# adri-romsor/iterative_inference_segm

Measured on AMD Instinct MI355X. Metric: refined images/s (FCN-8 + standard DAE, 10-step iterative inference, 224x224, 11 classes), higher is better.
Workload: dtype f32; 1 GPU; BASELINE configs[1]: FCN-8 + standard DAE (f64c1p2, pool4, trackind, skip), 224x224x3, batch 64/GPU, 10 steps, step 0.1, early stop off; per batch: pred_fcn_fn, val_fn, pred_dae_fn+val_fn, refine, val_fn; global_batch=64, parallelism=dp1

## Files before the change

include/iiseg.h:

```cpp
#ifndef IISEG_H
#define IISEG_H

#include <stdint.h>

#ifdef __cplusplus
extern "C" {
#endif

typedef enum iiseg_status {
    IISEG_OK = 0,
    IISEG_ERR_NULL = -1,
    IISEG_ERR_SHAPE = -2,
    IISEG_ERR_ALIGN = -3,
    IISEG_ERR_LAUNCH = -4,
    IISEG_ERR_UNSUPPORTED = -5
} iiseg_status;

const char* iiseg_strerror(int status);
const char* iiseg_last_hip_error(void);
int iiseg_abi_version(void);
const char* iiseg_target_arch(void);

int iiseg_profile_begin(int capacity);
int iiseg_profile_count(void);
// ... 34 lines not shown
                        const float* pre, const float* pooled, const float* wp, const int32_t* ktab,
                        const float* bias, const float* add, float* out, float* pool_out);

int iiseg_conv_mask_supported(const iiseg_conv_desc* d);
int iiseg_conv_mask_f32(void* stream, const iiseg_conv_desc* d, const float* x1, const float* x2,
                        const float* pre, const float* pooled, const uint8_t* mask_in,
                        const float* wp, const int32_t* ktab, const float* bias, const float* add,
                        float* out, float* pool_out, uint8_t* mask_out);

int iiseg_conv_halo_seam(int on);
int64_t iiseg_conv_halo_seam_launches(void);

int iiseg_conv_bnrelu_supported(const iiseg_conv_desc* d);
int iiseg_conv_bnrelu_f32(void* stream, const iiseg_conv_desc* d, const float* x, int64_t x_bstride,
                          const float* beta, const float* gamma, const float* mean,
                          const float* inv_std, const float* wp, const int32_t* ktab,
                          const float* bias, float* out);

#define IISEG_WINO_INPUT 1u
#define IISEG_WINO_GEMM 2u
#define IISEG_WINO_OUTPUT 4u
#define IISEG_WINO_ALL 7u
#define IISEG_WINO_FUSED 8u
int iiseg_conv_wino_supported(const iiseg_conv_desc* d);
int64_t iiseg_conv_wino_weight_elems(const iiseg_conv_desc* d);
int64_t iiseg_conv_wino_workspace_elems(const iiseg_conv_desc* d);
int iiseg_conv_wino_pack_f32(void* stream, const iiseg_conv_desc* d, const float* w,
                             int64_t stride_o, int64_t stride_c, float* U);
int iiseg_conv_wino_f32(void* stream, const iiseg_conv_desc* d, const float* x1, const float* x2,
                        const float* pre, const float* pooled, const float* U, const float* bias,
                        const float* add, float* workspace, float* out, uint32_t stages);
int iiseg_conv_wino_input_wide(int on);
int iiseg_conv_wino_input_path(const iiseg_conv_desc* d, int mask_bytes);
int iiseg_conv_wino_pool_supported(const iiseg_conv_desc* d);
int iiseg_conv_wino_mask_f32(void* stream, const iiseg_conv_desc* d, const float* x1, const float* x2,
                             const float* pre, const float* pooled, const uint8_t* mask_in,
                             const float* U, const float* bias, const float* add, float* workspace,
                             float* out, float* pool_out, uint8_t* mask_out, uint32_t stages);

int iiseg_conv_wino_bf16_supported(const iiseg_conv_desc* d);
int64_t iiseg_conv_wino_bf16_weight_bytes(const iiseg_conv_desc* d);
int64_t iiseg_conv_wino_bf16_workspace_bytes(const iiseg_conv_desc* d);
int iiseg_conv_wino_bf16_pack(void* stream, const iiseg_conv_desc* d, const float* w,
                              int64_t stride_o, int64_t stride_c, void* U16);
int iiseg_conv_wino_bf16(void* stream, const iiseg_conv_desc* d, const float* x1, const float* x2,
                         const float* pre, const float* pooled, const void* U16, const float* bias,
                         const float* add, void* workspace, float* out, uint32_t stages);

int iiseg_conv_gemm_bf16_supported(const iiseg_conv_desc* d);
int64_t iiseg_conv_gemm_bf16_weight_bytes(const iiseg_conv_desc* d);
int64_t iiseg_conv_gemm_bf16_workspace_bytes(const iiseg_conv_desc* d);
int iiseg_conv_gemm_bf16_pack(void* stream, const iiseg_conv_desc* d, const float* w,
                              int64_t stride_o, int64_t stride_c, void* U16);
int iiseg_conv_gemm_bf16(void* stream, const iiseg_conv_desc* d, const float* x, const void* U16,
                         const float* bias, void* workspace, float* out);

int iiseg_conv_halo_bf16_supported(const iiseg_conv_desc* d);
int64_t iiseg_conv_halo_bf16_weight_bytes(const iiseg_conv_desc* d);
int iiseg_conv_halo_bf16_pack(void* stream, const iiseg_conv_desc* d, const float* w,
                              int64_t stride_o, int64_t stride_c, void* wp16);
int iiseg_conv_halo_bf16(void* stream, const iiseg_conv_desc* d, const float* x1, const float* x2,
                         const float* pre, const float* pooled, const void* wp16, const float* bias,
                         const float* add, float* out, float* pool_out, const uint8_t* mask_in,
                         uint8_t* mask_out);

int iiseg_conv_wino_f64_supported(const iiseg_conv_desc* d);
// ... 335 lines not shown
```

iterative_inference_segm_amd/_lib.py:

```python
import ctypes as C
import os

HERE = os.path.dirname(os.path.abspath(__file__))
LIB_PATH = os.path.join(HERE, 'libiiseg_hip.so')

ABI_VERSION = 34

CONV_RELU = 1
CONV_UNPOOL = 2
CONV_X3 = 8
CONV_TRANSPOSED2 = 4
CONV_ZINS = 16


class ConvDesc(C.Structure):
    _fields_ = [(n, C.c_int32) for n in
                ('B', 'C1', 'C2', 'H', 'W', 'Cout', 'KH', 'KW', 'pad', 'dil',
                 'oy0', 'ox0', 'OH', 'OW', 'AH', 'AW', 'ay0', 'ax0')] + \
               [('flags', C.c_uint32), ('Kpad', C.c_int32), ('Mpad', C.c_int32),
                ('out_ctot', C.c_int32), ('out_c0', C.c_int32),
                ('out_H', C.c_int32), ('out_W', C.c_int32), ('out_y0', C.c_int32),
                ('out_x0', C.c_int32), ('tile_y0', C.c_int32), ('tile_x0', C.c_int32)]


# ... 43 lines not shown


_vp, _i32, _i64, _f32, _f64 = C.c_void_p, C.c_int32, C.c_int64, C.c_float, C.c_double

SIGNATURES = {
    'iiseg_strerror': (C.c_char_p, [C.c_int]),
    'iiseg_last_hip_error': (C.c_char_p, []),
    'iiseg_abi_version': (C.c_int, []),
    'iiseg_profile_begin': (C.c_int, [C.c_int]),
    'iiseg_profile_count': (C.c_int, []),
    'iiseg_profile_end': (C.c_int, [C.POINTER(C.c_float), C.c_int]),
    'iiseg_target_arch': (C.c_char_p, []),
    'iiseg_conv_ktab_entries': (C.c_int, [C.POINTER(ConvDesc)]),
    'iiseg_conv_plan': (C.c_int, [C.POINTER(ConvDesc)]),
    'iiseg_conv_pack_f32': (C.c_int, [_vp, C.POINTER(ConvDesc), _vp, _i64, _i64, _vp, _vp]),
    'iiseg_conv_f32': (C.c_int, [_vp, C.POINTER(ConvDesc)] + [_vp] * 9),
    'iiseg_conv_small_supported': (C.c_int, [C.POINTER(ConvDesc)]),
    'iiseg_conv_pool_supported': (C.c_int, [C.POINTER(ConvDesc)]),
    'iiseg_conv_pool_f32': (C.c_int, [_vp, C.POINTER(ConvDesc)] + [_vp] * 10),
    'iiseg_conv_halo_seam': (C.c_int, [C.c_int]),
    'iiseg_conv_halo_seam_launches': (_i64, []),
    'iiseg_conv_mask_supported': (C.c_int, [C.POINTER(ConvDesc)]),
    'iiseg_conv_mask_f32': (C.c_int, [_vp, C.POINTER(ConvDesc)] + [_vp] * 12),
    'iiseg_conv_bnrelu_supported': (C.c_int, [C.POINTER(ConvDesc)]),
    'iiseg_conv_bnrelu_f32': (C.c_int, [_vp, C.POINTER(ConvDesc), _vp, _i64] + [_vp] * 8),
    'iiseg_conv_wino_supported': (C.c_int, [C.POINTER(ConvDesc)]),
    'iiseg_conv_wino_weight_elems': (_i64, [C.POINTER(ConvDesc)]),
    'iiseg_conv_wino_workspace_elems': (_i64, [C.POINTER(ConvDesc)]),
    'iiseg_conv_wino_pack_f32': (C.c_int, [_vp, C.POINTER(ConvDesc), _vp, _i64, _i64, _vp]),
    'iiseg_conv_wino_f32': (C.c_int, [_vp, C.POINTER(ConvDesc)] + [_vp] * 9 + [C.c_uint32]),
    'iiseg_conv_wino_pool_supported': (C.c_int, [C.POINTER(ConvDesc)]),
    'iiseg_conv_wino_input_wide': (C.c_int, [C.c_int]),
    'iiseg_conv_wino_input_path': (C.c_int, [C.POINTER(ConvDesc), C.c_int]),
    'iiseg_conv_wino_mask_f32': (C.c_int, [_vp, C.POINTER(ConvDesc)] + [_vp] * 12 + [C.c_uint32]),
    'iiseg_conv_wino_bf16_supported': (C.c_int, [C.POINTER(ConvDesc)]),
    'iiseg_conv_wino_bf16_weight_bytes': (_i64, [C.POINTER(ConvDesc)]),
    'iiseg_conv_wino_bf16_workspace_bytes': (_i64, [C.POINTER(ConvDesc)]),
    'iiseg_conv_wino_bf16_pack': (C.c_int, [_vp, C.POINTER(ConvDesc), _vp, _i64, _i64, _vp]),
    'iiseg_conv_wino_bf16': (C.c_int, [_vp, C.POINTER(ConvDesc)] + [_vp] * 9 + [C.c_uint32]),
    'iiseg_conv_gemm_bf16_supported': (C.c_int, [C.POINTER(ConvDesc)]),
    'iiseg_conv_gemm_bf16_weight_bytes': (_i64, [C.POINTER(ConvDesc)]),
    'iiseg_conv_gemm_bf16_workspace_bytes': (_i64, [C.POINTER(ConvDesc)]),
    'iiseg_conv_gemm_bf16_pack': (C.c_int, [_vp, C.POINTER(ConvDesc), _vp, _i64, _i64, _vp]),
    'iiseg_conv_gemm_bf16': (C.c_int, [_vp, C.POINTER(ConvDesc)] + [_vp] * 5),
    'iiseg_conv_halo_bf16_supported': (C.c_int, [C.POINTER(ConvDesc)]),
    'iiseg_conv_halo_bf16_weight_bytes': (_i64, [C.POINTER(ConvDesc)]),
    'iiseg_conv_halo_bf16_pack': (C.c_int, [_vp, C.POINTER(ConvDesc), _vp, _i64, _i64, _vp]),
    'iiseg_conv_halo_bf16': (C.c_int, [_vp, C.POINTER(ConvDesc)] + [_vp] * 11),
    'iiseg_conv_wino_f64_supported': (C.c_int, [C.POINTER(ConvDesc)]),
    'iiseg_conv_wino_f64_weight_elems': (_i64, [C.POINTER(ConvDesc)]),
    'iiseg_conv_wino_f64_workspace_elems': (_i64, [C.POINTER(ConvDesc)]),
    'iiseg_conv_wino_pack_f64': (C.c_int, [_vp, C.POINTER(ConvDesc), _vp, _i64, _i64, _vp]),
    'iiseg_conv_wino_f64': (C.c_int, [_vp, C.POINTER(ConvDesc)] + [_vp] * 9),
    'iiseg_conv_c8_supported': (C.c_int, [C.POINTER(ConvDesc)]),
    'iiseg_conv_c8_is_flat': (C.c_int, [C.POINTER(ConvDesc)]),
    'iiseg_conv_c8_force_tiling': (C.c_int, [C.c_int, C.c_int, C.c_int]),
    'iiseg_conv_c8_tiling': (C.c_int, [C.POINTER(ConvDesc), C.c_int, C.POINTER(C.c_int32)]),
    'iiseg_conv_c8': (C.c_int, [_vp, C.POINTER(ConvDesc)] + [_vp] * 6 + [_i32, _vp, _i32, _vp, _vp]),
    'iiseg_conv_c8_slice': (C.c_int, [_vp, C.POINTER(ConvDesc), _vp, _i32] + [_vp] * 5 + [_i32, _vp, _i32, _vp, _vp]),
    'iiseg_unpool_c8': (C.c_int, [_vp] * 4 + [C.c_int] * 7),
    'iiseg_conv_c8_m16_supported': (C.c_int, [C.POINTER(ConvDesc)]),
    'iiseg_conv_c8_m16': (C.c_int, [_vp, C.POINTER(ConvDesc), _vp, _i32] + [_vp] * 6 + [_i32]),
    'iiseg_conv_c8_m16_workspace_bytes': (_i64, [C.POINTER(ConvDesc)]),
    'iiseg_conv_c8_m16_ws': (C.c_int, [_vp, C.POINTER(ConvDesc), _vp, _i32] + [_vp] * 6 + [_i32, _vp, _i64, _vp, _vp, _f64] + [_vp] * 4 + [_i32]),
    'iiseg_conv1x1_c8_weight_bytes': (_i64, [C.c_int, C.c_int]),
    'iiseg_conv1x1_c8_pack': (C.c_int, [_vp, _vp, _i64, _i64, C.c_int, C.c_int, C.c_int, _vp]),
# ... 145 lines not shown
```

iterative_inference_segm_amd/csrc/conv_wino.hip:

```cpp
#include <hip/hip_runtime.h>
#include <stdint.h>
#include <stdlib.h>
#include <atomic>
#include <type_traits>
#include "iiseg.h"
#include "common.h"
#include "conv_common.h"

using namespace iiseg;

namespace {

struct WinoParams {
    const float* x1;
    const float* x2;
    const float* pre;
    const float* pooled;
    const uint8_t* mask_in;
    int h2, w2;
    const float* U;
    const float* bias;
    const float* add;
    float* V;
    float* M;
// ... 574 lines not shown
                for (int j = 0; j < TN; ++j)
                    acc[i][j] = __builtin_amdgcn_mfma_f32_32x32x2f32(a[ch & 1][i], b[ch & 1][j],
                                                                     acc[i][j], 0, 0, 0);
            if constexpr (ch == 0) {
                if (more) WINO_STAGE(kt + NBUF - 1, sbuf)
            }
            __builtin_amdgcn_sched_barrier(0);
        });
        if (NBUF == 3 && more) {
            WINO_WAIT_ONE_STAGE_IN_FLIGHT()
        } else {
            asm volatile("s_waitcnt vmcnt(0)" ::: "memory");
        }
        __syncthreads();
        if (++buf == NBUF) buf = 0;
    }
#undef WINO_STAGE
#undef WINO_WAIT_ONE_STAGE_IN_FLIGHT

    float* Mx = p.M + (size_t)xi * p.Mpad * p.Tpad;
#pragma unroll
    for (int j = 0; j < TN; ++j) {
        const int t = t0 + wn * WTN + j * 32 + l31;
#pragma unroll
        for (int i = 0; i < TM; ++i)
#pragma unroll
            for (int r = 0; r < 16; ++r) {
                const int co = m0 + wm * WTM + i * 32 + (r & 3) + 8 * (r >> 2) + 4 * lh;
                Mx[(size_t)co * p.Tpad + t] = acc[i][j][r];
            }
    }
}

template <int BM, int BN, int WM, int WN, int BK, int MINW>
__global__ __launch_bounds__(WM * WN * 64, MINW) void wino_fused_kernel(const WinoParams p) {
    constexpr int NCH = BK / 2;
    constexpr int WTM = BM / WM, WTN = BN / WN;
    constexpr int TM = WTM / 32, TN = WTN / 32;
    constexpr int NT = WM * WN * 64;
    constexpr int AV = BK * BM / 4, BV = BK * BN / 4;
    constexpr int APT = AV / NT, BPT = BV / NT;
    static_assert(AV % NT == 0 && BV % NT == 0, "tile config");

    __shared__ __attribute__((aligned(16))) float As[2][BK][BM];
    __shared__ __attribute__((aligned(16))) float Bs[2][BK][BN];

    int tt, mt;
    tile_of_block(blockIdx.x, gridDim.x, p.n_ttiles, p.n_mtiles, tt, mt);
    const int m0 = mt * BM, t0 = tt * BN;
    const int tid = threadIdx.x, lane = tid & 63, wave = tid >> 6;
    const int wm = wave / WN, wn = wave % WN;
    const int l31 = lane & 31, lh = lane >> 5;
    const int nkt = p.Kc / BK;
    const size_t ustride = (size_t)p.Kc * p.Mpad, vstride = (size_t)p.Kc * p.Tpad;
    const int ubytes = p.Kc * p.Mpad * 4, vbytes = p.Kc * p.Tpad * 4;

#define WINO_STAGE(XI, KT, BUF)                                                                    \
    {                                                                                              \
        const __amdgpu_buffer_rsrc_t ar = mk_rsrc(p.U + (size_t)(XI) * ustride, ubytes);           \
        const __amdgpu_buffer_rsrc_t br = mk_rsrc(p.V + (size_t)(XI) * vstride, vbytes);           \
        static_for<0, APT>([&](auto J) __attribute__((always_inline)) {                            \
            constexpr int j = decltype(J)::value;                                                  \
            const int f = j * NT + tid;                                                            \
            const int row = f / (BM / 4), c4 = f % (BM / 4);                                       \
            __builtin_amdgcn_raw_ptr_buffer_load_lds(                                              \
                ar, (__attribute__((address_space(3))) void*)(&As[BUF][0][0] + (j * NT + wave * 64) * 4), \
                16, (int)(4u * (unsigned)(((KT) * BK + row) * p.Mpad + m0 + c4 * 4)), 0, 0, 0);    \
        });                                                                                        \
        static_for<0, BPT>([&](auto J) __attribute__((always_inline)) {                            \
            constexpr int j = decltype(J)::value;                                                  \
            const int f = j * NT + tid;                                                            \
            const int row = f / (BN / 4), c4 = f % (BN / 4);                                       \
            __builtin_amdgcn_raw_ptr_buffer_load_lds(                                              \
                br, (__attribute__((address_space(3))) void*)(&Bs[BUF][0][0] + (j * NT + wave * 64) * 4), \
                16, (int)(4u * (unsigned)(((KT) * BK + row) * p.Tpad + t0 + c4 * 4)), 0, 0, 0);    \
        });                                                                                        \
    }

    f32x16 acc[TM][TN], Y[4][TM][TN];
#pragma unroll
    for (int i = 0; i < TM; ++i)
#pragma unroll
        for (int j = 0; j < TN; ++j)
#pragma unroll
            for (int r = 0; r < 16; ++r) {
                acc[i][j][r] = 0.f;
                Y[0][i][j][r] = Y[1][i][j][r] = Y[2][i][j][r] = Y[3][i][j][r] = 0.f;
            }

    WINO_STAGE(0, 0, 0)
    asm volatile("s_waitcnt vmcnt(0)" ::: "memory");
    __syncthreads();

    int xi = 0, kt = 0;
    const int total = 16 * nkt;
    for (int s = 0; s < total; ++s) {
        const int buf = s & 1;
        int nxi = xi, nkt1 = kt + 1;
        if (nkt1 == nkt) { nkt1 = 0; ++nxi; }
        const bool more = s + 1 < total;
        float a[2][TM], b[2][TN];
#pragma unroll
        for (int i = 0; i < TM; ++i) a[0][i] = As[buf][lh][wm * WTM + i * 32 + l31];
#pragma unroll
        for (int j = 0; j < TN; ++j) b[0][j] = Bs[buf][lh][wn * WTN + j * 32 + l31];
        static_for<0, NCH>([&](auto CH) __attribute__((always_inline)) {
            constexpr int ch = decltype(CH)::value;
            if constexpr (ch + 1 < NCH) {
                const int kk = (ch + 1) * 2 + lh;
#pragma unroll
                for (int i = 0; i < TM; ++i) a[(ch + 1) & 1][i] = As[buf][kk][wm * WTM + i * 32 + l31];
#pragma unroll
                for (int j = 0; j < TN; ++j) b[(ch + 1) & 1][j] = Bs[buf][kk][wn * WTN + j * 32 + l31];
            }
#pragma unroll
            for (int i = 0; i < TM; ++i)
#pragma unroll
                for (int j = 0; j < TN; ++j)
                    acc[i][j] = __builtin_amdgcn_mfma_f32_32x32x2f32(a[ch & 1][i], b[ch & 1][j],
                                                                     acc[i][j], 0, 0, 0);
            if constexpr (ch == 0) {
                if (more) WINO_STAGE(nxi, nkt1, buf ^ 1)
            }
            __builtin_amdgcn_sched_barrier(0);
        });
        if (nkt1 == 0) {
            const int wi = xi >> 2, wj = xi & 3;
            const float r0 = wi < 3 ? 1.f : 0.f, r1 = wi == 0 ? 0.f : (wi == 1 ? 1.f : -1.f);
            const float c0 = wj < 3 ? 1.f : 0.f, c1 = wj == 0 ? 0.f : (wj == 1 ? 1.f : -1.f);
            const float k00 = r0 * c0, k01 = r0 * c1, k10 = r1 * c0, k11 = r1 * c1;
#define WINO_FOLD(Q, KQ)                                                                            \
            if ((KQ) != 0.f) {                                                                      \
                _Pragma("unroll") for (int i = 0; i < TM; ++i)                                      \
                _Pragma("unroll") for (int j = 0; j < TN; ++j)                                      \
                _Pragma("unroll") for (int r = 0; r < 16; ++r)                                      \
                    Y[Q][i][j][r] = fmaf((KQ), acc[i][j][r], Y[Q][i][j][r]);                        \
            }
            WINO_FOLD(0, k00)
            WINO_FOLD(1, k01)
            WINO_FOLD(2, k10)
            WINO_FOLD(3, k11)
#undef WINO_FOLD
#pragma unroll
            for (int i = 0; i < TM; ++i)
#pragma unroll
                for (int j = 0; j < TN; ++j)
#pragma unroll
                    for (int r = 0; r < 16; ++r) acc[i][j][r] = 0.f;
        }
        xi = nxi;
        kt = nkt1;
        asm volatile("s_waitcnt vmcnt(0)" ::: "memory");
        __syncthreads();
    }
#undef WINO_STAGE

    typedef float f32x2u __attribute__((ext_vector_type(2), aligned(4)));
    const int ntt = p.nty * p.ntx;
    const size_t OPL = (size_t)p.out_H * p.out_W, APL = (size_t)p.AH * p.AW;
    float* Lbias = &As[0][0][0];
    for (int f = tid; f < BM; f += NT) Lbias[f] = (p.bias && m0 + f < p.Cout) ? p.bias[m0 + f] : 0.f;
    __syncthreads();
    float bias_r[TM][16];
#pragma unroll
    for (int i = 0; i < TM; ++i)
#pragma unroll
        for (int r = 0; r < 16; ++r) bias_r[i][r] = Lbias[wm * WTM + i * 32 + (r & 3) + 8 * (r >> 2) + 4 * lh];
#pragma unroll
    for (int j = 0; j < TN; ++j) {
        const int t = t0 + wn * WTN + j * 32 + l31;
        if (t >= p.T) continue;
        const int b = t / ntt;
        const int rr = t - b * ntt;
        const int tyl = rr / p.ntx, txl = rr - tyl * p.ntx;
        const int wy = p.ty0 + 2 * tyl - p.oy0, wx = p.tx0 + 2 * txl - p.ox0;
        const bool rok[2] = {(unsigned)wy < (unsigned)p.OH, (unsigned)(wy + 1) < (unsigned)p.OH};
        const bool cok[2] = {(unsigned)wx < (unsigned)p.OW, (unsigned)(wx + 1) < (unsigned)p.OW};
        const bool pair = cok[0] && cok[1];
        const bool whole = p.pool && rok[1] && cok[1];
        float* ob = p.out ? p.out + ((size_t)b * p.out_ctot + p.out_c0) * OPL +
                                (ptrdiff_t)(p.out_y0 + wy) * p.out_W + p.out_x0 + wx
                          : nullptr;
        const float* ab = p.add ? p.add + (size_t)b * p.Cout * APL +
                                      (ptrdiff_t)(p.ay0 + wy) * p.AW + p.ax0 + wx
                                : nullptr;
#pragma unroll
        for (int i = 0; i < TM; ++i)
// ... 139 lines not shown
        d->pad < 0 || d->OH <= 0 || d->OW <= 0 || d->oy0 < 0 || d->ox0 < 0)
        return IISEG_ERR_SHAPE;
    const int fullH = d->H + 2 * d->pad - 2, fullW = d->W + 2 * d->pad - 2;
    if (d->oy0 + d->OH > fullH || d->ox0 + d->OW > fullW) return IISEG_ERR_SHAPE;
    if ((d->C1 + d->C2) % 16) return IISEG_ERR_UNSUPPORTED;
    g.Kc = d->C1 + d->C2;
    g.bm = d->Cout > 128 ? 256 : (d->Cout > 64 ? 128 : 64);
    g.Mpad = round_up(d->Cout, g.bm);
    if ((d->tile_y0 | d->tile_x0) & ~1) return IISEG_ERR_SHAPE;
    g.ty0 = d->oy0 - ((d->oy0 - d->tile_y0) & 1);
    g.tx0 = d->ox0 - ((d->ox0 - d->tile_x0) & 1);
    g.nty = (d->oy0 + d->OH - g.ty0 + 1) >> 1;
    g.ntx = (d->ox0 + d->OW - g.tx0 + 1) >> 1;
    const int64_t T = (int64_t)d->B * g.nty * g.ntx;
    const int64_t Tpad = (T + 127) / 128 * 128;
    if (Tpad * g.Kc * 4 >= (int64_t)1 << 31 || (int64_t)g.Kc * g.Mpad * 4 >= (int64_t)1 << 31)
        return IISEG_ERR_UNSUPPORTED;
    g.T = (int)T;
    g.Tpad = (int)Tpad;
    return IISEG_OK;
}

std::atomic<int> g_input_wide{-1};

int input_wide_setting() {
    int v = g_input_wide.load();
    if (v < 0) {
        v = getenv("IISEG_WINO_INPUT_WIDE") ? (atoi(getenv("IISEG_WINO_INPUT_WIDE")) != 0) : 1;
        g_input_wide.store(v);
    }
    return v;
}

bool iw_fits(const WinoParams& p, int nt) {
    const int NC = 2 * p.ntx + 2;
    for (int t0 = 0; t0 < p.T; t0 += 4 * nt) {
        const int t1 = t0 + 4 * nt < p.T ? t0 + 4 * nt : p.T;
        if ((int64_t)iw_chunk(t0, t1, p.ntx, p.nty).NR * NC > (int64_t)IW_E * nt) return false;
    }
    return true;
}

int ilds_nt(const WinoParams& p);
constexpr int IW_NT = 256;

int iw_shape(const WinoParams& p, bool unpool, bool mb) {
    const int setting = input_wide_setting();
    if (!setting || (unpool && !mb)) return 0;
    if (setting != 2) {
        if (p.T < 4096) return 0;
        const int lnt = mb ? 0 : ilds_nt(p);
        if (lnt && (p.nty * p.ntx) % lnt == 0) return 0;
    }
    const int64_t HW = (int64_t)p.H * p.W, cmax = p.C1 > p.C2 ? p.C1 : p.C2;
    if (HW > (1 << IW_PBITS) || (int64_t)p.B * cmax * HW >= (int64_t)1 << 30) return 0;
    const int64_t waves1 = ((int64_t)p.T + 255) / 256 * p.Kc;
    int ch = 8;
    if (p.Kc % 32 == 0 && waves1 / 32 >= 2048) ch = 32;
    else if (waves1 / 16 >= 2048) ch = 16;
    return iw_fits(p, IW_NT) ? ch : 0;
}

int ilds_nt(const WinoParams& p) {
    static const int lds = getenv("IISEG_WINO_INPUT_LDS") ? atoi(getenv("IISEG_WINO_INPUT_LDS")) : 1;
    const int ntt = p.nty * p.ntx;
    int nt = 0;
// ... 18 lines not shown
    }
    const int nt = ilds_nt(p);
    const int ntt = p.nty * p.ntx;
    if (nt) {
        const int chunks = (ntt + nt - 1) / nt;
        const dim3 g2(p.B * chunks, p.Kc / ILDS_CH);
#define WINO_ILDS(U, N, ...) IISEG_LAUNCH((wino_input_lds_kernel<U, N, ##__VA_ARGS__>), g2, dim3(N), 0, s, p, chunks)
        if (mb) { if (nt == 256) WINO_ILDS(true, 256, true); else if (nt == 128) WINO_ILDS(true, 128, true); else WINO_ILDS(true, 64, true); }
        else if (unpool) { if (nt == 256) WINO_ILDS(true, 256); else if (nt == 128) WINO_ILDS(true, 128); else WINO_ILDS(true, 64); }
        else { if (nt == 256) WINO_ILDS(false, 256); else if (nt == 128) WINO_ILDS(false, 128); else WINO_ILDS(false, 64); }
#undef WINO_ILDS
        return;
    }
    const int nc = unpool ? ICH / 2 : ICH;
    const dim3 grid((p.T + 255) / 256, (p.Kc + nc - 1) / nc), block(256);
    if (!unpool) {
        IISEG_LAUNCH((wino_input_kernel<false, 0, 0>), grid, block, 0, s, p);
        return;
    }
    const int py = (p.ty0 - p.pad) & 1, px = (p.tx0 - p.pad) & 1;
    if (mb) {
        if (py && px) IISEG_LAUNCH((wino_input_kernel<true, 1, 1, true>), grid, block, 0, s, p);
        else if (py) IISEG_LAUNCH((wino_input_kernel<true, 1, 0, true>), grid, block, 0, s, p);
        else if (px) IISEG_LAUNCH((wino_input_kernel<true, 0, 1, true>), grid, block, 0, s, p);
        else IISEG_LAUNCH((wino_input_kernel<true, 0, 0, true>), grid, block, 0, s, p);
        return;
    }
    if (py && px) IISEG_LAUNCH((wino_input_kernel<true, 1, 1>), grid, block, 0, s, p);
    else if (py) IISEG_LAUNCH((wino_input_kernel<true, 1, 0>), grid, block, 0, s, p);
    else if (px) IISEG_LAUNCH((wino_input_kernel<true, 0, 1>), grid, block, 0, s, p);
    else IISEG_LAUNCH((wino_input_kernel<true, 0, 0>), grid, block, 0, s, p);
}

}

int iiseg_wino_output_launch(hipStream_t s, const iiseg_conv_desc* d, const float* M, int Mpad,
                             int Tpad, const float* bias, const float* add, float* out) {
    WinoParams p = {};
    p.M = const_cast<float*>(M);
    p.bias = bias; p.add = add; p.out = out;
    p.B = d->B; p.Cout = d->Cout; p.pad = d->pad;
    p.oy0 = d->oy0; p.ox0 = d->ox0; p.OH = d->OH; p.OW = d->OW;
    p.ty0 = d->oy0 - ((d->oy0 - d->tile_y0) & 1);
    p.tx0 = d->ox0 - ((d->ox0 - d->tile_x0) & 1);
    p.nty = (d->oy0 + d->OH - p.ty0 + 1) >> 1;
    p.ntx = (d->ox0 + d->OW - p.tx0 + 1) >> 1;
    p.T = d->B * p.nty * p.ntx;
    p.Tpad = Tpad; p.Mpad = Mpad;
    p.AH = d->AH; p.AW = d->AW; p.ay0 = d->ay0; p.ax0 = d->ax0;
    p.relu = (d->flags & IISEG_CONV_RELU) ? 1 : 0;
    p.out_ctot = d->out_ctot > 0 ? d->out_ctot : d->Cout;
    p.out_c0 = d->out_ctot > 0 ? d->out_c0 : 0;
    p.out_H = d->out_H > 0 ? d->out_H : d->OH;
    p.out_W = d->out_H > 0 ? d->out_W : d->OW;
    p.out_y0 = d->out_H > 0 ? d->out_y0 : 0;
    p.out_x0 = d->out_H > 0 ? d->out_x0 : 0;
    IISEG_LAUNCH(wino_output_kernel, dim3((p.T + 255) / 256, (d->Cout + OCH - 1) / OCH),
                       dim3(256), 0, s, p);
    return iiseg_check_launch();
}

extern "C" int iiseg_conv_wino_supported(const iiseg_conv_desc* d) {
    WinoGeom g;
    return wino_geom(d, g) == IISEG_OK ? 1 : 0;
}

extern "C" int iiseg_conv_wino_input_wide(int on) {
    if (on >= 0) g_input_wide.store(on > 1 ? 2 : on);
    return input_wide_setting();
}

extern "C" int iiseg_conv_wino_input_path(const iiseg_conv_desc* d, int mask_bytes) {
    WinoGeom g;
    const int st = wino_geom(d, g);
    if (st) return st;
    WinoParams p = {};
    const bool unpool = (d->flags & IISEG_CONV_UNPOOL) != 0;
    if (mask_bytes && !unpool) return IISEG_ERR_UNSUPPORTED;
    p.B = d->B; p.C1 = d->C1; p.C2 = d->C2; p.H = d->H; p.W = d->W;
    p.nty = g.nty; p.ntx = g.ntx; p.T = g.T; p.Tpad = g.Tpad; p.Kc = g.Kc;
    if (iw_shape(p, unpool, mask_bytes != 0)) return 2;
    return ilds_nt(p) ? 1 : 0;
}

extern "C" int64_t iiseg_conv_wino_weight_elems(const iiseg_conv_desc* d) {
    WinoGeom g;
    if (wino_geom(d, g) != IISEG_OK) return 0;
    return (int64_t)16 * g.Kc * g.Mpad;
}

extern "C" int64_t iiseg_conv_wino_workspace_elems(const iiseg_conv_desc* d) {
    WinoGeom g;
    if (wino_geom(d, g) != IISEG_OK) return 0;
    return (int64_t)16 * g.Tpad * ((int64_t)g.Kc + g.Mpad);
}

extern "C" int iiseg_conv_wino_pack_f32(void* stream, const iiseg_conv_desc* d, const float* w,
                                        int64_t stride_o, int64_t stride_c, float* U) {
    WinoGeom g;
    const int st = wino_geom(d, g);
    if (st) return st;
    if (!w || !U) return IISEG_ERR_NULL;
    const int64_t n = (int64_t)g.Kc * g.Mpad;
    const int grid = (int)((n + 255) / 256 < 4096 ? (n + 255) / 256 : 4096);
    IISEG_LAUNCH(wino_weight_kernel, dim3(grid), dim3(256), 0, (hipStream_t)stream, w,
                       stride_o, stride_c, U, d->C1 + d->C2, d->Cout, g.Kc, g.Mpad);
    return iiseg_check_launch();
}

static bool wino_pool_ok(const iiseg_conv_desc* d) {
    WinoGeom g;
    if (wino_geom(d, g) != IISEG_OK) return false;
    const int fullH = d->H + 2 * d->pad - 2, fullW = d->W + 2 * d->pad - 2;
    if ((d->tile_y0 | d->tile_x0 | d->oy0 | d->ox0) & 1) return false;
    if ((d->OH & 1) && d->oy0 + d->OH != fullH) return false;
// ... 35 lines not shown
    p.U = U;
    p.bias = bias;
    p.add = add;
    p.V = workspace;
    p.M = workspace + (size_t)16 * g.Kc * g.Tpad;
    p.out = out;
    p.B = d->B; p.C1 = d->C1; p.C2 = d->C2; p.H = d->H; p.W = d->W;
    p.Cout = d->Cout; p.pad = d->pad;
    p.oy0 = d->oy0; p.ox0 = d->ox0; p.OH = d->OH; p.OW = d->OW;
    p.ty0 = g.ty0; p.tx0 = g.tx0; p.nty = g.nty; p.ntx = g.ntx;
    p.T = g.T; p.Tpad = g.Tpad; p.Kc = g.Kc; p.Mpad = g.Mpad;
    p.AH = d->AH; p.AW = d->AW; p.ay0 = d->ay0; p.ax0 = d->ax0;
    if (add && (d->ay0 < 0 || d->ax0 < 0 || d->ay0 + d->OH > d->AH || d->ax0 + d->OW > d->AW))
        return IISEG_ERR_SHAPE;
    p.relu = (d->flags & IISEG_CONV_RELU) ? 1 : 0;
    p.out_ctot = d->out_ctot > 0 ? d->out_ctot : d->Cout;
    p.out_c0 = d->out_ctot > 0 ? d->out_c0 : 0;
    if (p.out_c0 < 0 || p.out_c0 + d->Cout > p.out_ctot) return IISEG_ERR_SHAPE;
    p.out_H = d->out_H > 0 ? d->out_H : d->OH;
    p.out_W = d->out_H > 0 ? d->out_W : d->OW;
    p.out_y0 = d->out_H > 0 ? d->out_y0 : 0;
    p.out_x0 = d->out_H > 0 ? d->out_x0 : 0;
    if (p.out_y0 < 0 || p.out_x0 < 0 || p.out_y0 + d->OH > p.out_H || p.out_x0 + d->OW > p.out_W)
        return IISEG_ERR_SHAPE;
    p.n_ttiles = g.Tpad / 128;
    p.n_mtiles = g.Mpad / g.bm;
    hipStream_t s = (hipStream_t)stream;
    const int tb = (g.T + 255) / 256;
    if (stages & IISEG_WINO_FUSED) {
        if (g.Kc % 32) return IISEG_ERR_UNSUPPORTED;
        if (stages & IISEG_WINO_INPUT)
            launch_wino_input(s, p, unpool);
        if (stages & IISEG_WINO_GEMM) {
            if (g.bm == 64) {
                p.n_mtiles = g.Mpad / 64;
                IISEG_LAUNCH((wino_fused_kernel<64, 128, 1, 4, 32, 2>),
                                   dim3(p.n_ttiles * p.n_mtiles), dim3(256), 0, s, p);
                return iiseg_check_launch();
            }
            p.n_mtiles = g.Mpad / 128;
            const int w0 = p.n_ttiles * p.n_mtiles, w2 = (g.Tpad / 64) * p.n_mtiles;
            const double cost0 = (w0 + 255) / 256, cost2 = 0.5 * 1.03 * ((w2 + 255) / 256);
            static const int bk64 = getenv("IISEG_WINO_FUSED_BK") ? atoi(getenv("IISEG_WINO_FUSED_BK")) == 64 : 0;
            const bool big = bk64 && g.Kc % 64 == 0;
            if (g.Kc <= 128 || cost2 < cost0) {
                p.n_ttiles = g.Tpad / 64;
                if (big)
                    IISEG_LAUNCH((wino_fused_kernel<128, 64, 2, 2, 64, 2>),
                                       dim3(p.n_ttiles * p.n_mtiles), dim3(256), 0, s, p);
                else
                IISEG_LAUNCH((wino_fused_kernel<128, 64, 2, 2, 32, 2>),
                                   dim3(p.n_ttiles * p.n_mtiles), dim3(256), 0, s, p);
            } else if (big)
                IISEG_LAUNCH((wino_fused_kernel<128, 128, 2, 4, 64, 2>),
                                   dim3(p.n_ttiles * p.n_mtiles), dim3(512), 0, s, p);
            else
            IISEG_LAUNCH((wino_fused_kernel<128, 128, 2, 4, 32, 2>),
                               dim3(p.n_ttiles * p.n_mtiles), dim3(512), 0, s, p);
        }
        return iiseg_check_launch();
    }
    if (stages & IISEG_WINO_INPUT)
        launch_wino_input(s, p, unpool);
    const int grid = 16 * p.n_ttiles * p.n_mtiles;
    if (stages & IISEG_WINO_GEMM) {
        static const int nbuf = getenv("IISEG_WINO_NBUF") ? atoi(getenv("IISEG_WINO_NBUF")) : 2;
        int bm = g.bm;
        if (bm == 64) {
            IISEG_LAUNCH((wino_gemm_kernel<64, 128, 1, 4, 2>), dim3(grid), dim3(256), 0, s, p);
            bm = 0;
        }
        if (bm == 256) {
            const int w256 = grid, w128 = 2 * grid;
            if (0.5 * 1.06 * ((w128 + 255) / 256) < (double)((w256 + 255) / 256)) bm = 128;
        }
        const int grid2 = bm ? 16 * p.n_ttiles * (g.Mpad / bm) : 0;
        if (bm) p.n_mtiles = g.Mpad / bm;
        static const int bk32 = getenv("IISEG_WINO_GEMM_BK") ? atoi(getenv("IISEG_WINO_GEMM_BK")) == 32 : 0;
        if (bm && bk32 && g.Kc % 32 == 0 && nbuf != 3) {
            if (bm == 256)
                IISEG_LAUNCH((wino_gemm_kernel<256, 128, 4, 2, 2, 32>), dim3(grid), dim3(512), 0, s, p);
            else
                IISEG_LAUNCH((wino_gemm_kernel<128, 128, 2, 2, 2, 32>), dim3(grid2), dim3(256), 0, s, p);
        } else
        if (bm == 0) {
        } else if (bm == 256 && nbuf == 3)
            IISEG_LAUNCH((wino_gemm_kernel<256, 128, 4, 2, 3>), dim3(grid), dim3(512), 0, s, p);
        else if (bm == 256)
            IISEG_LAUNCH((wino_gemm_kernel<256, 128, 4, 2, 2>), dim3(grid), dim3(512), 0, s, p);
        else if (nbuf == 3)
            IISEG_LAUNCH((wino_gemm_kernel<128, 128, 2, 2, 3>), dim3(grid2), dim3(256), 0, s, p);
// ... 169 lines not shown
```

iterative_inference_segm_amd/ops.py:

```python
import collections
import ctypes as C
import os

import torch

from . import _lib
from ._lib import ConvDesc, DeconvDesc, CONV_RELU, CONV_UNPOOL, CONV_TRANSPOSED2, CONV_X3, CONV_ZINS, check

CONV_PROFILE = None
CONV_PROFILE_INFO = None
KERNEL_BYTES = {}

_SUFFIX = {torch.float32: 'f32', torch.float64: 'f64'}

WINO_MIN_CIN = int(os.environ.get('IISEG_WINO_MIN_CIN', '128'))
WINO_F64 = os.environ.get('IISEG_WINO_F64', '1') != '0'
WINO_F64_MIN_CIN = int(os.environ.get('IISEG_WINO_F64_MIN_CIN', '128'))
WINO_F64_MIN_COUT = int(os.environ.get('IISEG_WINO_F64_MIN_COUT', '128'))
WINO_MIN_COUT = int(os.environ.get('IISEG_WINO_MIN_COUT', '128'))
WINO_FUSED_MAX_CIN = int(os.environ.get('IISEG_WINO_FUSED_MAX_CIN', '256'))
POOL_FUSE = os.environ.get('IISEG_POOL_FUSE', '1') != '0'
WINO_POOL_FUSE = os.environ.get('IISEG_WINO_POOL_FUSE', '1') != '0'
F64_POOL_FUSE = os.environ.get('IISEG_F64_POOL_FUSE', '1') != '0'
F64_MASKS = os.environ.get('IISEG_F64_MASKS', '1') != '0'
# ... 16 lines not shown
        with open(BF16_PICKS_FILE) as f:
            return {k: v for k, v in json.load(f).get('picks', {}).items() if v in ('wino', 'halo')}
    except OSError:
        return {}


BF16_PICKS = _load_bf16_picks()
BF16_TIMES = {}


def _bf16_static_pick(Cin, OW):
    fill = OW / (32.0 * ((OW + 31) // 32))
    return 'wino' if (Cin >= 1024 or fill < 0.7) else 'halo'


C8_M16 = os.environ.get('IISEG_C8_M16', '1') != '0'
BF16_UPCONV1 = os.environ.get('IISEG_BF16_UPCONV1', '0') != '0'
BF16_WINO_MIN_COUT = int(os.environ.get('IISEG_BF16_WINO_MIN_COUT', '256'))
_SCRATCH_KINDS = {'f32': torch.float32, 'f64': torch.float64, 'bn': torch.float64, 'm16': torch.uint8}
_scratch = {}
_ws_tag = [0]


def halo_seam(on=None):
    return bool(_lib.load().iiseg_conv_halo_seam(-1 if on is None else int(bool(on))))


def halo_seam_launches():
    return int(_lib.load().iiseg_conv_halo_seam_launches())


def wino_input_wide(on=None, force=False):
    return bool(_lib.load().iiseg_conv_wino_input_wide(-1 if on is None else (2 if on and force else int(bool(on)))))


class workspace_tag:

    def __init__(self, tag):
        self.tag, self.prev = tag, None

    def __enter__(self):
        self.prev, _ws_tag[0] = _ws_tag[0], self.tag
        return self

    def __exit__(self, *exc):
        _ws_tag[0] = self.prev
        return False


def current_workspace_tag():
    return _ws_tag[0]


def _workspace(kind, n, device):
    key = (kind, device, _ws_tag[0])
    ws = _scratch.get(key)
    if ws is None or ws.numel() < n:
        _scratch[key] = None
        ws = _scratch[key] = torch.empty(int(n), dtype=_SCRATCH_KINDS[kind], device=device)
    return ws


def drop_workspaces(tag):
    for key in [k for k in _scratch if k[2] == tag]:
        _scratch.pop(key, None)

# ... 1672 lines not shown
```

Before: 529.9 images/s.

## Add configurable multi-buffer ring and precomputed DMA offsets to fused Winograd kernel

Measured after the change: 532.6 images/s (median of 6 runs). Within noise of the previous version (+0.5%).

```diff
diff --git a/include/iiseg.h b/include/iiseg.h
--- a/include/iiseg.h
+++ b/include/iiseg.h
@@ -90,6 +90,7 @@
                         const float* add, float* workspace, float* out, uint32_t stages);
 int iiseg_conv_wino_input_wide(int on);
 int iiseg_conv_wino_input_path(const iiseg_conv_desc* d, int mask_bytes);
+int iiseg_conv_wino_fused_ring(int ring);
 int iiseg_conv_wino_pool_supported(const iiseg_conv_desc* d);
 int iiseg_conv_wino_mask_f32(void* stream, const iiseg_conv_desc* d, const float* x1, const float* x2,
                              const float* pre, const float* pooled, const uint8_t* mask_in,
diff --git a/iterative_inference_segm_amd/_lib.py b/iterative_inference_segm_amd/_lib.py
--- a/iterative_inference_segm_amd/_lib.py
+++ b/iterative_inference_segm_amd/_lib.py
@@ -99,6 +99,7 @@
     'iiseg_conv_wino_pool_supported': (C.c_int, [C.POINTER(ConvDesc)]),
     'iiseg_conv_wino_input_wide': (C.c_int, [C.c_int]),
     'iiseg_conv_wino_input_path': (C.c_int, [C.POINTER(ConvDesc), C.c_int]),
+    'iiseg_conv_wino_fused_ring': (C.c_int, [C.c_int]),
     'iiseg_conv_wino_mask_f32': (C.c_int, [_vp, C.POINTER(ConvDesc)] + [_vp] * 12 + [C.c_uint32]),
     'iiseg_conv_wino_bf16_supported': (C.c_int, [C.POINTER(ConvDesc)]),
     'iiseg_conv_wino_bf16_weight_bytes': (_i64, [C.POINTER(ConvDesc)]),
diff --git a/iterative_inference_segm_amd/csrc/conv_wino.hip b/iterative_inference_segm_amd/csrc/conv_wino.hip
--- a/iterative_inference_segm_amd/csrc/conv_wino.hip
+++ b/iterative_inference_segm_amd/csrc/conv_wino.hip
@@ -630,7 +630,7 @@
     }
 }
 
-template <int BM, int BN, int WM, int WN, int BK, int MINW>
+template <int BM, int BN, int WM, int WN, int BK, int MINW, int NBUF = 2>
 __global__ __launch_bounds__(WM * WN * 64, MINW) void wino_fused_kernel(const WinoParams p) {
     constexpr int NCH = BK / 2;
     constexpr int WTM = BM / WM, WTN = BN / WN;
@@ -639,9 +639,11 @@
     constexpr int AV = BK * BM / 4, BV = BK * BN / 4;
     constexpr int APT = AV / NT, BPT = BV / NT;
     static_assert(AV % NT == 0 && BV % NT == 0, "tile config");
-
-    __shared__ __attribute__((aligned(16))) float As[2][BK][BM];
-    __shared__ __attribute__((aligned(16))) float Bs[2][BK][BN];
+    constexpr int OPS = APT + BPT;
+    static_assert(NBUF >= 2 && NBUF - 1 <= 16 && (NBUF - 2) * OPS <= 63, "ring config");
+
+    __shared__ __attribute__((aligned(16))) float As[NBUF][BK][BM];
+    __shared__ __attribute__((aligned(16))) float Bs[NBUF][BK][BN];
 
     int tt, mt;
     tile_of_block(blockIdx.x, gridDim.x, p.n_ttiles, p.n_mtiles, tt, mt);
@@ -653,26 +655,30 @@
     const size_t ustride = (size_t)p.Kc * p.Mpad, vstride = (size_t)p.Kc * p.Tpad;
     const int ubytes = p.Kc * p.Mpad * 4, vbytes = p.Kc * p.Tpad * 4;
 
+    unsigned avo[APT], bvo[BPT];
+#pragma unroll
+    for (int j = 0; j < APT; ++j) {
+        const int f = j * NT + tid;
+        avo[j] = 4u * (unsigned)((f / (BM / 4)) * p.Mpad + m0 + (f % (BM / 4)) * 4);
+    }
+#pragma unroll
+    for (int j = 0; j < BPT; ++j) {
+        const int f = j * NT + tid;
+        bvo[j] = 4u * (unsigned)((f / (BN / 4)) * p.Tpad + t0 + (f % (BN / 4)) * 4);
+    }
+    const unsigned lds_a = __builtin_amdgcn_readfirstlane(lds_addr(&As[0][0][0]) + (unsigned)wave * 1024u);
+    const unsigned lds_b = __builtin_amdgcn_readfirstlane(lds_addr(&Bs[0][0][0]) + (unsigned)wave * 1024u);
 #define WINO_STAGE(XI, KT, BUF)                                                                    \
     {                                                                                              \
-        const __amdgpu_buffer_rsrc_t ar = mk_rsrc(p.U + (size_t)(XI) * ustride, ubytes);           \
-        const __amdgpu_buffer_rsrc_t br = mk_rsrc(p.V + (size_t)(XI) * vstride, vbytes);           \
-        static_for<0, APT>([&](auto J) __attribute__((always_inline)) {                            \
-            constexpr int j = decltype(J)::value;                                                  \
-            const int f = j * NT + tid;                                                            \
-            const int row = f / (BM / 4), c4 = f % (BM / 4);                                       \
-            __builtin_amdgcn_raw_ptr_buffer_load_lds(                                              \
-                ar, (__attribute__((address_space(3))) void*)(&As[BUF][0][0] + (j * NT + wave * 64) * 4), \
-                16, (int)(4u * (unsigned)(((KT) * BK + row) * p.Mpad + m0 + c4 * 4)), 0, 0, 0);    \
-        });                                                                                        \
-        static_for<0, BPT>([&](auto J) __attribute__((always_inline)) {                            \
-            constexpr int j = decltype(J)::value;                                                  \
-            const int f = j * NT + tid;                                                            \
-            const int row = f / (BN / 4), c4 = f % (BN / 4);                                       \
-            __builtin_amdgcn_raw_ptr_buffer_load_lds(                                              \
-                br, (__attribute__((address_space(3))) void*)(&Bs[BUF][0][0] + (j * NT + wave * 64) * 4), \
-                16, (int)(4u * (unsigned)(((KT) * BK + row) * p.Tpad + t0 + c4 * 4)), 0, 0, 0);    \
-        });                                                                                        \
+        const i32x4s ar = mk_srsrc(p.U + (size_t)(XI) * ustride, (unsigned)ubytes);                \
+        const i32x4s br = mk_srsrc(p.V + (size_t)(XI) * vstride, (unsigned)vbytes);                \
+        const unsigned soa = __builtin_amdgcn_readfirstlane(4u * (unsigned)((KT) * BK * p.Mpad));  \
+        const unsigned sob = __builtin_amdgcn_readfirstlane(4u * (unsigned)((KT) * BK * p.Tpad));  \
+        const unsigned la = __builtin_amdgcn_readfirstlane(lds_a + (unsigned)(BUF) * (BK * BM * 4)); \
+        const unsigned lb = __builtin_amdgcn_readfirstlane(lds_b + (unsigned)(BUF) * (BK * BN * 4)); \
+        asm volatile("s_nop 4");      \
+        _Pragma("unroll") for (int j = 0; j < APT; ++j) dma16(ar, la + j * NT * 16, avo[j], soa);  \
+        _Pragma("unroll") for (int j = 0; j < BPT; ++j) dma16(br, lb + j * NT * 16, bvo[j], sob);  \
     }
 
     f32x16 acc[TM][TN], Y[4][TM][TN];
@@ -686,17 +692,25 @@
                 Y[0][i][j][r] = Y[1][i][j][r] = Y[2][i][j][r] = Y[3][i][j][r] = 0.f;
             }
 
-    WINO_STAGE(0, 0, 0)
-    asm volatile("s_waitcnt vmcnt(0)" ::: "memory");
+    int sxi = 0, skt = 0;
+#define WINO_STAGE_NEXT(BUF)                                                                       \
+    {                                                                                              \
+        WINO_STAGE(sxi, skt, BUF)                                                                  \
+        if (++skt == nkt) { skt = 0; ++sxi; }                                                      \
+    }
+    static_for<0, NBUF - 1>([&](auto SLOT) __attribute__((always_inline)) {
+        constexpr int slot = decltype(SLOT)::value;
+        WINO_STAGE_NEXT(slot)
+    });
+    asm volatile("s_waitcnt vmcnt(%0)" ::"n"((NBUF - 2) * OPS) : "memory");
     __syncthreads();
 
-    int xi = 0, kt = 0;
+    int xi = 0, kt = 0, buf = 0;
     const int total = 16 * nkt;
     for (int s = 0; s < total; ++s) {
-        const int buf = s & 1;
-        int nxi = xi, nkt1 = kt + 1;
-        if (nkt1 == nkt) { nkt1 = 0; ++nxi; }
-        const bool more = s + 1 < total;
+        const bool more = s + NBUF - 1 < total;
+        int sbuf = buf + NBUF - 1;
+        if (sbuf >= NBUF) sbuf -= NBUF;
         float a[2][TM], b[2][TN];
 #pragma unroll
         for (int i = 0; i < TM; ++i) a[0][i] = As[buf][lh][wm * WTM + i * 32 + l31];
@@ -718,11 +732,11 @@
                     acc[i][j] = __builtin_amdgcn_mfma_f32_32x32x2f32(a[ch & 1][i], b[ch & 1][j],
                                                                      acc[i][j], 0, 0, 0);
             if constexpr (ch == 0) {
-                if (more) WINO_STAGE(nxi, nkt1, buf ^ 1)
+                if (more) WINO_STAGE_NEXT(sbuf)
             }
             __builtin_amdgcn_sched_barrier(0);
         });
-        if (nkt1 == 0) {
+        if (++kt == nkt) {
             const int wi = xi >> 2, wj = xi & 3;
             const float r0 = wi < 3 ? 1.f : 0.f, r1 = wi == 0 ? 0.f : (wi == 1 ? 1.f : -1.f);
             const float c0 = wj < 3 ? 1.f : 0.f, c1 = wj == 0 ? 0.f : (wj == 1 ? 1.f : -1.f);
@@ -745,12 +759,15 @@
                 for (int j = 0; j < TN; ++j)
 #pragma unroll
                     for (int r = 0; r < 16; ++r) acc[i][j][r] = 0.f;
-        }
-        xi = nxi;
-        kt = nkt1;
-        asm volatile("s_waitcnt vmcnt(0)" ::: "memory");
+            kt = 0;
+            ++xi;
+        }
+        if (NBUF > 2 && more) asm volatile("s_waitcnt vmcnt(%0)" ::"n"((NBUF - 2) * OPS) : "memory");
+        else asm volatile("s_waitcnt vmcnt(0)" ::: "memory");
         __syncthreads();
-    }
+        if (++buf == NBUF) buf = 0;
+    }
+#undef WINO_STAGE_NEXT
 #undef WINO_STAGE
 
     typedef float f32x2u __attribute__((ext_vector_type(2), aligned(4)));
@@ -956,6 +973,20 @@
     return v;
 }
 
+std::atomic<int> g_fused_ring{-1};
+
+int fused_ring_setting() {
+    int v = g_fused_ring.load();
+    if (v < 0) {
+        v = getenv("IISEG_WINO_FUSED_RING") ? atoi(getenv("IISEG_WINO_FUSED_RING")) : 0;
+        if (v < 2 || v > 4) v = 0;
+        g_fused_ring.store(v);
+    }
+    return v;
+}
+
+int fused_ring_form(int setting) { return setting ? setting : 2; }
+
 bool iw_fits(const WinoParams& p, int nt) {
     const int NC = 2 * p.ntx + 2;
     for (int t0 = 0; t0 < p.T; t0 += 4 * nt) {
@@ -1076,6 +1107,11 @@
 extern "C" int iiseg_conv_wino_input_wide(int on) {
     if (on >= 0) g_input_wide.store(on > 1 ? 2 : on);
     return input_wide_setting();
+}
+
+extern "C" int iiseg_conv_wino_fused_ring(int ring) {
+    if (ring >= 0) g_fused_ring.store(ring >= 2 && ring <= 4 ? ring : 0);
+    return fused_ring_setting();
 }
 
 extern "C" int iiseg_conv_wino_input_path(const iiseg_conv_desc* d, int mask_bytes) {
@@ -1190,10 +1226,17 @@
         if (stages & IISEG_WINO_INPUT)
             launch_wino_input(s, p, unpool);
         if (stages & IISEG_WINO_GEMM) {
+#define WINO_FUSED(BM, BN, WM, WN, NTHR)                                                           \
+            {                                                                                      \
+                const int ring = fused_ring_form(fused_ring_setting());                            \
+                const dim3 fg(p.n_ttiles * p.n_mtiles);                                            \
+                if (ring == 3) IISEG_LAUNCH((wino_fused_kernel<BM, BN, WM, WN, 32, 2, 3>), fg, dim3(NTHR), 0, s, p); \
+                else if (ring == 4) IISEG_LAUNCH((wino_fused_kernel<BM, BN, WM, WN, 16, 2, 4>), fg, dim3(NTHR), 0, s, p); \
+                else IISEG_LAUNCH((wino_fused_kernel<BM, BN, WM, WN, 32, 2>), fg, dim3(NTHR), 0, s, p); \
+            }
             if (g.bm == 64) {
                 p.n_mtiles = g.Mpad / 64;
-                IISEG_LAUNCH((wino_fused_kernel<64, 128, 1, 4, 32, 2>),
-                                   dim3(p.n_ttiles * p.n_mtiles), dim3(256), 0, s, p);
+                WINO_FUSED(64, 128, 1, 4, 256)
                 return iiseg_check_launch();
             }
             p.n_mtiles = g.Mpad / 128;
@@ -1207,14 +1250,13 @@
                     IISEG_LAUNCH((wino_fused_kernel<128, 64, 2, 2, 64, 2>),
                                        dim3(p.n_ttiles * p.n_mtiles), dim3(256), 0, s, p);
                 else
-                IISEG_LAUNCH((wino_fused_kernel<128, 64, 2, 2, 32, 2>),
-                                   dim3(p.n_ttiles * p.n_mtiles), dim3(256), 0, s, p);
+                    WINO_FUSED(128, 64, 2, 2, 256)
             } else if (big)
                 IISEG_LAUNCH((wino_fused_kernel<128, 128, 2, 4, 64, 2>),
                                    dim3(p.n_ttiles * p.n_mtiles), dim3(512), 0, s, p);
             else
-            IISEG_LAUNCH((wino_fused_kernel<128, 128, 2, 4, 32, 2>),
-                               dim3(p.n_ttiles * p.n_mtiles), dim3(512), 0, s, p);
+                WINO_FUSED(128, 128, 2, 4, 512)
+#undef WINO_FUSED
         }
         return iiseg_check_launch();
     }
diff --git a/iterative_inference_segm_amd/ops.py b/iterative_inference_segm_amd/ops.py
--- a/iterative_inference_segm_amd/ops.py
+++ b/iterative_inference_segm_amd/ops.py
@@ -72,6 +72,10 @@
 
 def wino_input_wide(on=None, force=False):
     return bool(_lib.load().iiseg_conv_wino_input_wide(-1 if on is None else (2 if on and force else int(bool(on)))))
+
+
+def wino_fused_ring(ring=None):
+    return int(_lib.load().iiseg_conv_wino_fused_ring(-1 if ring is None else int(ring)))
 
 
 class workspace_tag:
```

## Add 32-wide-tile fused Winograd GEMM variants with more waves, selectable at runtime

Applied to the files above, without the earlier changes.

Result: no change. 520.1 images/s before, 523.6 images/s after (median of 6 runs) (+0.7%).

```diff
diff --git a/include/iiseg.h b/include/iiseg.h
--- a/include/iiseg.h
+++ b/include/iiseg.h
@@ -90,6 +90,10 @@
                         const float* add, float* workspace, float* out, uint32_t stages);
 int iiseg_conv_wino_input_wide(int on);
 int iiseg_conv_wino_input_path(const iiseg_conv_desc* d, int mask_bytes);
+#define IISEG_WINO_FUSED_VARIANT_W32 4
+#define IISEG_WINO_FUSED_VARIANT_BK64 8
+int iiseg_conv_wino_fused_w32(int on);
+int iiseg_conv_wino_fused_variant(const iiseg_conv_desc* d);
 int iiseg_conv_wino_pool_supported(const iiseg_conv_desc* d);
 int iiseg_conv_wino_mask_f32(void* stream, const iiseg_conv_desc* d, const float* x1, const float* x2,
                              const float* pre, const float* pooled, const uint8_t* mask_in,
diff --git a/iterative_inference_segm_amd/_lib.py b/iterative_inference_segm_amd/_lib.py
--- a/iterative_inference_segm_amd/_lib.py
+++ b/iterative_inference_segm_amd/_lib.py
@@ -99,6 +99,8 @@
     'iiseg_conv_wino_pool_supported': (C.c_int, [C.POINTER(ConvDesc)]),
     'iiseg_conv_wino_input_wide': (C.c_int, [C.c_int]),
     'iiseg_conv_wino_input_path': (C.c_int, [C.POINTER(ConvDesc), C.c_int]),
+    'iiseg_conv_wino_fused_w32': (C.c_int, [C.c_int]),
+    'iiseg_conv_wino_fused_variant': (C.c_int, [C.POINTER(ConvDesc)]),
     'iiseg_conv_wino_mask_f32': (C.c_int, [_vp, C.POINTER(ConvDesc)] + [_vp] * 12 + [C.c_uint32]),
     'iiseg_conv_wino_bf16_supported': (C.c_int, [C.POINTER(ConvDesc)]),
     'iiseg_conv_wino_bf16_weight_bytes': (_i64, [C.POINTER(ConvDesc)]),
diff --git a/iterative_inference_segm_amd/csrc/conv_wino.hip b/iterative_inference_segm_amd/csrc/conv_wino.hip
--- a/iterative_inference_segm_amd/csrc/conv_wino.hip
+++ b/iterative_inference_segm_amd/csrc/conv_wino.hip
@@ -639,6 +639,7 @@
     constexpr int AV = BK * BM / 4, BV = BK * BN / 4;
     constexpr int APT = AV / NT, BPT = BV / NT;
     static_assert(AV % NT == 0 && BV % NT == 0, "tile config");
+    constexpr bool OPAQUE_DMA = TM * TN == 1;
 
     __shared__ __attribute__((aligned(16))) float As[2][BK][BM];
     __shared__ __attribute__((aligned(16))) float Bs[2][BK][BN];
@@ -653,6 +654,7 @@
     const size_t ustride = (size_t)p.Kc * p.Mpad, vstride = (size_t)p.Kc * p.Tpad;
     const int ubytes = p.Kc * p.Mpad * 4, vbytes = p.Kc * p.Tpad * 4;
 
+    typedef __attribute__((address_space(3))) float* lds_fp;
 #define WINO_STAGE(XI, KT, BUF)                                                                    \
     {                                                                                              \
         const __amdgpu_buffer_rsrc_t ar = mk_rsrc(p.U + (size_t)(XI) * ustride, ubytes);           \
@@ -661,16 +663,20 @@
             constexpr int j = decltype(J)::value;                                                  \
             const int f = j * NT + tid;                                                            \
             const int row = f / (BM / 4), c4 = f % (BM / 4);                                       \
+            lds_fp dst = (lds_fp)(&As[BUF][0][0] + (j * NT + wave * 64) * 4);                      \
+            if constexpr (OPAQUE_DMA) asm volatile("" : "+v"(dst));                                \
             __builtin_amdgcn_raw_ptr_buffer_load_lds(                                              \
-                ar, (__attribute__((address_space(3))) void*)(&As[BUF][0][0] + (j * NT + wave * 64) * 4), \
+                ar, (__attribute__((address_space(3))) void*)dst,                                  \
                 16, (int)(4u * (unsigned)(((KT) * BK + row) * p.Mpad + m0 + c4 * 4)), 0, 0, 0);    \
         });                                                                                        \
         static_for<0, BPT>([&](auto J) __attribute__((always_inline)) {                            \
             constexpr int j = decltype(J)::value;                                                  \
             const int f = j * NT + tid;                                                            \
             const int row = f / (BN / 4), c4 = f % (BN / 4);                                       \
+            lds_fp dst = (lds_fp)(&Bs[BUF][0][0] + (j * NT + wave * 64) * 4);                      \
+            if constexpr (OPAQUE_DMA) asm volatile("" : "+v"(dst));                                \
             __builtin_amdgcn_raw_ptr_buffer_load_lds(                                              \
-                br, (__attribute__((address_space(3))) void*)(&Bs[BUF][0][0] + (j * NT + wave * 64) * 4), \
+                br, (__attribute__((address_space(3))) void*)dst,                                  \
                 16, (int)(4u * (unsigned)(((KT) * BK + row) * p.Tpad + t0 + c4 * 4)), 0, 0, 0);    \
         });                                                                                        \
     }
@@ -1040,6 +1046,35 @@
     else IISEG_LAUNCH((wino_input_kernel<true, 0, 0>), grid, block, 0, s, p);
 }
 
+std::atomic<int> g_fused_w32{-1};
+
+int fused_w32_setting() {
+    int v = g_fused_w32.load();
+    if (v < 0) {
+        const int e = getenv("IISEG_WINO_FUSED_W32") ? atoi(getenv("IISEG_WINO_FUSED_W32")) : 1;
+        v = e > 1 ? 2 : (e != 0);
+        g_fused_w32.store(v);
+    }
+    return v;
+}
+
+enum { FV_64x128 = 0, FV_128x64 = 1, FV_128x128 = 2, FV_W32 = 4, FV_BK64 = 8 };
+
+int fused_variant(const WinoGeom& g) {
+    const int setting = fused_w32_setting();
+    const int w32 = setting ? FV_W32 : 0;
+    if (g.bm == 64) return FV_64x128 | w32;
+    const int n_mtiles = g.Mpad / 128;
+    const int w0 = (g.Tpad / 128) * n_mtiles, w2 = (g.Tpad / 64) * n_mtiles;
+    const double cost0 = (w0 + 255) / 256, cost2 = 0.5 * 1.03 * ((w2 + 255) / 256);
+    const bool narrow_w64 = g.Kc <= 128 || cost2 < cost0;
+    static const int bk64 = getenv("IISEG_WINO_FUSED_BK") ? atoi(getenv("IISEG_WINO_FUSED_BK")) == 64 : 0;
+    if (bk64 && g.Kc % 64 == 0) return (narrow_w64 ? FV_128x64 : FV_128x128) | FV_BK64;
+    static const int bn = getenv("IISEG_WINO_FUSED_BN") ? atoi(getenv("IISEG_WINO_FUSED_BN")) : 0;
+    const bool narrow = bn == 64 || (bn != 128 && (setting == 1 || narrow_w64));
+    return (narrow ? FV_128x64 : FV_128x128) | w32;
+}
+
 }
 
 int iiseg_wino_output_launch(hipStream_t s, const iiseg_conv_desc* d, const float* M, int Mpad,
@@ -1089,6 +1124,19 @@
     p.nty = g.nty; p.ntx = g.ntx; p.T = g.T; p.Tpad = g.Tpad; p.Kc = g.Kc;
     if (iw_shape(p, unpool, mask_bytes != 0)) return 2;
     return ilds_nt(p) ? 1 : 0;
+}
+
+extern "C" int iiseg_conv_wino_fused_w32(int on) {
+    if (on >= 0) g_fused_w32.store(on > 1 ? 2 : on);
+    return fused_w32_setting();
+}
+
+extern "C" int iiseg_conv_wino_fused_variant(const iiseg_conv_desc* d) {
+    WinoGeom g;
+    const int st = wino_geom(d, g);
+    if (st) return st;
+    if (g.Kc % 32) return IISEG_ERR_UNSUPPORTED;
+    return fused_variant(g);
 }
 
 extern "C" int64_t iiseg_conv_wino_weight_elems(const iiseg_conv_desc* d) {
@@ -1190,31 +1238,25 @@
         if (stages & IISEG_WINO_INPUT)
             launch_wino_input(s, p, unpool);
         if (stages & IISEG_WINO_GEMM) {
-            if (g.bm == 64) {
-                p.n_mtiles = g.Mpad / 64;
-                IISEG_LAUNCH((wino_fused_kernel<64, 128, 1, 4, 32, 2>),
-                                   dim3(p.n_ttiles * p.n_mtiles), dim3(256), 0, s, p);
-                return iiseg_check_launch();
-            }
-            p.n_mtiles = g.Mpad / 128;
-            const int w0 = p.n_ttiles * p.n_mtiles, w2 = (g.Tpad / 64) * p.n_mtiles;
-            const double cost0 = (w0 + 255) / 256, cost2 = 0.5 * 1.03 * ((w2 + 255) / 256);
-            static const int bk64 = getenv("IISEG_WINO_FUSED_BK") ? atoi(getenv("IISEG_WINO_FUSED_BK")) == 64 : 0;
-            const bool big = bk64 && g.Kc % 64 == 0;
-            if (g.Kc <= 128 || cost2 < cost0) {
-                p.n_ttiles = g.Tpad / 64;
-                if (big)
-                    IISEG_LAUNCH((wino_fused_kernel<128, 64, 2, 2, 64, 2>),
-                                       dim3(p.n_ttiles * p.n_mtiles), dim3(256), 0, s, p);
-                else
-                IISEG_LAUNCH((wino_fused_kernel<128, 64, 2, 2, 32, 2>),
-                                   dim3(p.n_ttiles * p.n_mtiles), dim3(256), 0, s, p);
-            } else if (big)
-                IISEG_LAUNCH((wino_fused_kernel<128, 128, 2, 4, 64, 2>),
-                                   dim3(p.n_ttiles * p.n_mtiles), dim3(512), 0, s, p);
-            else
-            IISEG_LAUNCH((wino_fused_kernel<128, 128, 2, 4, 32, 2>),
-                               dim3(p.n_ttiles * p.n_mtiles), dim3(512), 0, s, p);
+            const int v = fused_variant(g);
+            const int bn = (v & 3) == FV_128x64 ? 64 : 128;
+            p.n_mtiles = g.Mpad / ((v & 3) == FV_64x128 ? 64 : 128);
+            p.n_ttiles = g.Tpad / bn;
+            const dim3 grid(p.n_ttiles * p.n_mtiles);
+#define WINO_FUSED(BM, BN, WM, WN, BK, MINW) \
+    IISEG_LAUNCH((wino_fused_kernel<BM, BN, WM, WN, BK, MINW>), grid, dim3(WM * WN * 64), 0, s, p)
+            switch (v) {
+                case FV_64x128: WINO_FUSED(64, 128, 1, 4, 32, 2); break;
+                case FV_64x128 | FV_W32: WINO_FUSED(64, 128, 2, 4, 32, 2); break;
+                case FV_128x64: WINO_FUSED(128, 64, 2, 2, 32, 2); break;
+                case FV_128x64 | FV_W32: WINO_FUSED(128, 64, 4, 2, 32, 2); break;
+                case FV_128x64 | FV_BK64: WINO_FUSED(128, 64, 2, 2, 64, 2); break;
+                case FV_128x128: WINO_FUSED(128, 128, 2, 4, 32, 2); break;
+                case FV_128x128 | FV_W32: WINO_FUSED(128, 128, 4, 4, 32, 1); break;
+                case FV_128x128 | FV_BK64: WINO_FUSED(128, 128, 2, 4, 64, 2); break;
+                default: return IISEG_ERR_UNSUPPORTED;
+            }
+#undef WINO_FUSED
         }
         return iiseg_check_launch();
     }
diff --git a/iterative_inference_segm_amd/ops.py b/iterative_inference_segm_amd/ops.py
--- a/iterative_inference_segm_amd/ops.py
+++ b/iterative_inference_segm_amd/ops.py
@@ -72,6 +72,10 @@
 
 def wino_input_wide(on=None, force=False):
     return bool(_lib.load().iiseg_conv_wino_input_wide(-1 if on is None else (2 if on and force else int(bool(on)))))
+
+
+def wino_fused_w32(on=None, width_rule=False):
+    return bool(_lib.load().iiseg_conv_wino_fused_w32(-1 if on is None else (2 if on and width_rule else int(bool(on)))))
 
 
 class workspace_tag:
```
